# De-Rosa/PPO-BipedalWalker

Measured on AMD Instinct MI355X. Metric: env-steps/sec (whole node) + PPO-update ms, 65k walkers at 1/2/4/8 MI355X, higher is better.
Workload: dtype f32; 1 GPU; BASELINE config 4: 65536 walkers over 1 GPU(s) (65536/GPU), config 3 step: rollout T_h=64 with policy sampling + PPO update E=5, global minibatch 65536 (65536/GPU); walkers_per_gpu=65536, global_walkers=65536, horizon=64, epochs=5, minibatch_global=65536, parallelism=dp1, exchange=none

## Files before the change

### ppo-bipedalwalker_amd/csrc/wk_device.h

```cpp
#pragma once
#include <float.h>
#include "wk_common.h"
#include "wk_sincos_small.h"


namespace wk {

#define DEV __device__ __forceinline__

struct V2 { float x, y; };
typedef float pf2 __attribute__((ext_vector_type(2)));
DEV V2 mk(float x, float y) { V2 r; r.x = x; r.y = y; return r; }
DEV V2 vadd(V2 a, V2 b) { return mk(a.x + b.x, a.y + b.y); }
DEV V2 vsub(V2 a, V2 b) { return mk(a.x - b.x, a.y - b.y); }
DEV V2 vmul(V2 a, float s) { return mk(a.x * s, a.y * s); }
DEV V2 vdiv(V2 a, float d) { float f = 1.0f / d; return mk(a.x * f, a.y * f); }
DEV V2 vneg(V2 a) { return mk(-a.x, -a.y); }
DEV float vdot(V2 a, V2 b) { return a.x * b.x + a.y * b.y; }
DEV float sqrt_core(float x) {
  const float y = __builtin_amdgcn_rsqf(x);
  const float s0 = x * y;
  const float e = __builtin_fmaf(-s0, s0, x);
  return __builtin_fmaf(e, 0.5f * y, s0);
}
// ... 270 lines not shown
  constexpr int steps = L == 16 ? 4 : (L == 8 ? 3 : 2);
#pragma unroll
  for (int s = 0; s < steps; s++) {
    const int osep = dpp_i(sep, s), oidx = dpp_i(idx, s);
    const float od = dpp_f(depth, s), onx = dpp_f(nx, s), ony = dpp_f(ny, s);
    sep |= osep;
    const bool take = (od < depth) || (od == depth && oidx < idx);
    depth = take ? od : depth;
    idx = take ? oidx : idx;
    nx = take ? onx : nx;
    ny = take ? ony : ny;
  }
}

template <int NA, int NB>
DEV void edge_of(const Poly<NA>& A, const Poly<NB>& B, int k, V2& p0, V2& p1) {
  uint32_t x0 = 0u, y0 = 0u, x1 = 0u, y1 = 0u;
#pragma unroll
  for (int i = 0; i < NA + NB; i++) {
    const uint32_t m = (k == i) ? 0xffffffffu : 0u;
    const bool fa = i < NA;
    const int a = fa ? i : i - NA;
    const int b = fa ? (a + 1) % NA : (a + 1) % NB;
    const float sx = fa ? A.x[fa ? a : 0] : B.x[fa ? 0 : a];
    const float sy = fa ? A.y[fa ? a : 0] : B.y[fa ? 0 : a];
    const float ex = fa ? A.x[fa ? b : 0] : B.x[fa ? 0 : b];
    const float ey = fa ? A.y[fa ? b : 0] : B.y[fa ? 0 : b];
    x0 |= m & __float_as_uint(sx); y0 |= m & __float_as_uint(sy);
    x1 |= m & __float_as_uint(ex); y1 |= m & __float_as_uint(ey);
  }
  p0 = mk(__uint_as_float(x0), __uint_as_float(y0));
  p1 = mk(__uint_as_float(x1), __uint_as_float(y1));
}

template <int L, int NA, int NB>
DEV bool sat_row(const Poly<NA>& A, const Poly<NB>& B, int sub, V2& normal, float& depth) {
  static_assert(NA + NB <= L, "one axis per lane");
  int sep = 0, idx = 1 << 20;
  float d = FLT_MAX, nx = 0.0f, ny = 0.0f;
  if (sub < NA + NB) {
    V2 p0, p1;
    edge_of(A, B, sub, p0, p1);
    const float ex = p1.x - p0.x, ey = p1.y - p0.y;
    V2 axis = mk(-ey, ex);
    if (!(axis.x == 0.0f && axis.y == 0.0f)) {
      axis = vnormalize(axis);
      float amin, amax, bmin, bmax;
      project2(axis.x, axis.y, A, B, amin, amax, bmin, bmax);
      float temp;
      bool overlapping;
      if (sub < NA) {
        temp = net_minf(bmax - amin, amax - bmin);
        overlapping = (amin < bmax) && (bmin < amax);
      } else {
        temp = net_minf(amax - bmin, bmax - amin);
        overlapping = (bmin < amax) && (amin < bmax);
      }
      if (!overlapping) sep = 1;
      d = temp; idx = sub; nx = axis.x; ny = axis.y;
    }
  }
  row_reduce<L>(sep, d, idx, nx, ny);
  normal = idx < (1 << 20) ? mk(nx, ny) : mk(0.0f, 0.0f);
  depth = d;
  const bool result = sep == 0;
  V2 dir = mk(B.cx - A.cx, B.cy - A.cy);
  if (vdot(dir, normal) > 0.0f) normal = vmul(normal, -1.0f);
  return result;
}

template <int N>
DEV V2 pick(const Poly<N>& p, int i) {
  uint32_t bx = 0u, by = 0u;
#pragma unroll
  for (int k = 0; k < N; k++) {
    const uint32_t m = (i == k) ? 0xffffffffu : 0u;
    bx |= m & __float_as_uint(p.x[k]);
    by |= m & __float_as_uint(p.y[k]);
  }
  return mk(__uint_as_float(bx), __uint_as_float(by));
}

DEV uint32_t bsel(uint32_t m, float a, uint32_t b) { return (m & __float_as_uint(a)) | (~m & b); }
template <int N, bool SAFE = false>
DEV void significant_face(const Poly<N>& P, V2 n, V2& fa, V2& fb, V2& fmax) {
  float mind = FLT_MAX;
  uint32_t sx = 0u, sy = 0u;
  uint32_t ax = __float_as_uint(P.x[0]), ay = __float_as_uint(P.y[0]);
  uint32_t bx = __float_as_uint(P.x[N - 2]), by = __float_as_uint(P.y[N - 2]);
#pragma unroll
  for (int i = 0; i < N; i++) {
    const float p = P.x[i] * n.x + P.y[i] * n.y;
    const bool lt = p < mind;
    const uint32_t m = lt ? 0xffffffffu : 0u;
    mind = lt ? p : mind;
    sx = bsel(m, P.x[i], sx);
    sy = bsel(m, P.y[i], sy);
    ax = bsel(m, P.x[(i + 1) % N], ax);
    ay = bsel(m, P.y[(i + 1) % N], ay);
    bx = bsel(m, P.x[(i + N - 1) % N], bx);
    by = bsel(m, P.y[(i + N - 1) % N], by);
  }
  const V2 sig = mk(__uint_as_float(sx), __uint_as_float(sy));
  const V2 va = mk(__uint_as_float(ax), __uint_as_float(ay));
  const V2 vb = mk(__uint_as_float(bx), __uint_as_float(by));
  V2 after = SAFE ? vnormalize(vsub(sig, va)) : vnormalize_edge(vsub(sig, va));
  V2 before = SAFE ? vnormalize(vsub(sig, vb)) : vnormalize_edge(vsub(sig, vb));
  const bool first = vdot(n, before) >= vdot(n, after);
  fa = first ? sig : va;
  fb = first ? vb : sig;
  fmax = sig;
}

template <int N>
DEV void significant_face_ax(const Poly<N>& P, const EdgeAxes<N>& AX, V2 n, V2& fa, V2& fb,
                             V2& fmax, V2& fdir) {
  float mind = FLT_MAX;
  uint32_t sx = 0u, sy = 0u;
  uint32_t ax = __float_as_uint(P.x[0]), ay = __float_as_uint(P.y[0]);
  uint32_t bx = __float_as_uint(P.x[N - 2]), by = __float_as_uint(P.y[N - 2]);
  uint32_t ex = __float_as_uint(AX.x[N - 1]), ey = __float_as_uint(AX.y[N - 1]);
  uint32_t px = __float_as_uint(AX.x[N - 2]), py = __float_as_uint(AX.y[N - 2]);
#pragma unroll
  for (int i = 0; i < N; i++) {
    const float p = P.x[i] * n.x + P.y[i] * n.y;
    const bool lt = p < mind;
    const uint32_t m = lt ? 0xffffffffu : 0u;
    mind = lt ? p : mind;
    sx = bsel(m, P.x[i], sx);
    sy = bsel(m, P.y[i], sy);
    ax = bsel(m, P.x[(i + 1) % N], ax);
    ay = bsel(m, P.y[(i + 1) % N], ay);
    bx = bsel(m, P.x[(i + N - 1) % N], bx);
    by = bsel(m, P.y[(i + N - 1) % N], by);
    ex = bsel(m, AX.x[i], ex);
    ey = bsel(m, AX.y[i], ey);
    px = bsel(m, AX.x[(i + N - 1) % N], px);
    py = bsel(m, AX.y[(i + N - 1) % N], py);
  }
  const V2 sig = mk(__uint_as_float(sx), __uint_as_float(sy));
  const V2 va = mk(__uint_as_float(ax), __uint_as_float(ay));
  const V2 vb = mk(__uint_as_float(bx), __uint_as_float(by));
  const V2 after = mk(-__uint_as_float(ey), __uint_as_float(ex));
  const V2 before = mk(__uint_as_float(py), -__uint_as_float(px));
  const bool first = vdot(n, before) >= vdot(n, after);
  fa = first ? sig : va;
  fb = first ? vb : sig;
  fmax = sig;
  fdir = first ? vneg(before) : after;
}
template <int N, int S>
DEV void significant_face_lds(const Poly<N>& P, const EdgeAxes<N>& AX, V2 n, float4* rec, V2& fa,
                              V2& fb, V2& fmax, V2& fdir) {
#pragma unroll
  for (int k = 0; k < N; k++) rec[k * S] = make_float4(P.x[k], P.y[k], AX.x[k], AX.y[k]);
  float mind = FLT_MAX;
  int idx = -1;
#pragma unroll
  for (int i = 0; i < N; i++) {
    const float p = P.x[i] * n.x + P.y[i] * n.y;
    const bool lt = p < mind;
    mind = lt ? p : mind;
    idx = lt ? i : idx;
  }
  const int ie = idx < 0 ? N - 1 : idx;
  const int inx = idx == N - 1 ? 0 : idx + 1;
  const int ipv = idx <= 0 ? idx + N - 1 : idx - 1;
  __builtin_amdgcn_wave_barrier();
  const float4 re = rec[ie * S], rn = rec[inx * S], rp = rec[ipv * S];
  const V2 sig = idx < 0 ? mk(0.0f, 0.0f) : mk(re.x, re.y);
  const V2 va = mk(rn.x, rn.y);
  const V2 vb = mk(rp.x, rp.y);
  const V2 after = mk(-re.w, re.z);
  const V2 before = mk(rp.w, -rp.z);
  const bool first = vdot(n, before) >= vdot(n, after);
  fa = first ? sig : va;
  fb = first ? vb : sig;
  fmax = sig;
  fdir = first ? vneg(before) : after;
}

DEV EdgeAxes<4> floor_axes() {
  EdgeAxes<4> a;
  a.x[0] = 1.0f;  a.y[0] = 0.0f;
  a.x[1] = -0.0f; a.y[1] = 1.0f;
  a.x[2] = -1.0f; a.y[2] = 0.0f;
  a.x[3] = -0.0f; a.y[3] = -1.0f;
  return a;
}

DEV int clip_vectors(V2 a, V2 b, V2 n, float offset, V2& o0, V2& o1) {
  const float da = vdot(a, n) - offset;
  const float db = vdot(b, n) - offset;
  const bool ka = da >= 0.0f, kb = db >= 0.0f, kx = da * db < 0.0f;
  const float location = da / (da - db);
  const V2 edge = vadd(vmul(vsub(b, a), location), a);
  const V2 second = kb ? b : edge;
  V2 r0 = ka ? a : (kb ? b : edge);
  V2 r1 = ka ? second : edge;
  const bool has0 = ka || kb || kx;
  const bool has1 = ka ? (kb || kx) : (kb && kx);
  o0 = has0 ? r0 : o0;
  o1 = has1 ? r1 : o1;
  return (int)ka + (int)kb + (int)kx;
}

DEV int contact_clip(V2 ra, V2 rb, V2 rmax, V2 rd, V2 ia, V2 ib, V2 imax, V2 id, V2 normal,
                     V2& c0, V2& c1) {
  V2 rf = vsub(rb, ra);
  V2 iv = vsub(ib, ia);
  if (fabsf(vdot(rf, normal)) > fabsf(vdot(iv, normal))) {
    V2 t;
    t = ra; ra = ia; ia = t;
    t = rb; rb = ib; ib = t;
    t = rmax; rmax = imax; imax = t;
    rd = id;
  }
  rf = rd;
  float offset = vdot(rf, ra);
  V2 p0 = mk(0.0f, 0.0f), p1 = mk(0.0f, 0.0f);
  const int k1 = clip_vectors(ia, ib, rf, offset, p0, p1);
  offset = vdot(rf, rb);
  V2 q0 = mk(0.0f, 0.0f), q1 = mk(0.0f, 0.0f);
  const int k2 = clip_vectors(p0, p1, vneg(rf), -offset, q0, q1);
  if (k1 < 2 || k2 < 2) return 0;
  V2 refn = mk(rf.y, -rf.x);
  float maximum = vdot(refn, rmax);
  int cnt = 2;
  if (vdot(refn, q0) - maximum < 0.0f) { q0 = q1; cnt = 1; }
  V2 last = cnt == 2 ? q1 : q0;
  if (vdot(refn, last) - maximum < 0.0f) cnt = cnt == 2 ? 1 : 0;
  c0 = q0;
  c1 = q1;
  return cnt;
}
template <int NA, int NB, int S = 0>
DEV int contact_points_ax(const Poly<NA>& A, const EdgeAxes<NA>& AXA, const Poly<NB>& B,
                          const EdgeAxes<NB>& AXB, V2 normal, V2& c0, V2& c1,
                          float4* rec = nullptr) {
  V2 ra, rb, rmax, rd, ia, ib, imax, id;
  if constexpr (S > 0) {
    significant_face_lds<NA, S>(A, AXA, normal, rec, ra, rb, rmax, rd);
    __builtin_amdgcn_wave_barrier();
    significant_face_lds<NB, S>(B, AXB, vneg(normal), rec, ia, ib, imax, id);
  } else {
    significant_face_ax(A, AXA, normal, ra, rb, rmax, rd);
    significant_face_ax(B, AXB, vneg(normal), ia, ib, imax, id);
  }
  return contact_clip(ra, rb, rmax, rd, ia, ib, imax, id, normal, c0, c1);
}
DEV void floor_face_ax(V2 n, V2& fa, V2& fb, V2& fmax, V2& fdir) {
  const float xa = -50.0f * n.x, xb = 1050.0f * n.x, ya = 1050.0f * n.y, yb = 900.0f * n.y;
  const float p[4] = {xa + ya, xa + yb, xb + yb, xb + ya};
  float mind = FLT_MAX;
  bool b0 = false, b1 = false;
#pragma unroll
  for (int i = 0; i < 4; i++) {
    const bool lt = p[i] < mind;
    mind = lt ? p[i] : mind;
    b0 = lt ? (i & 1) != 0 : b0;
    b1 = lt ? (i >> 1) != 0 : b1;
  }
  const bool bx = b0 != b1;
  const V2 sig = mk(b1 ? 1050.0f : -50.0f, bx ? 900.0f : 1050.0f);
  const V2 va = mk(bx ? 1050.0f : -50.0f, b1 ? 1050.0f : 900.0f);
  const V2 vb = mk(bx ? -50.0f : 1050.0f, b1 ? 900.0f : 1050.0f);
  const float ex = b0 ? -0.0f : (b1 ? -1.0f : 1.0f), ey = b0 ? (b1 ? -1.0f : 1.0f) : 0.0f;
  const float px = b0 ? (b1 ? -1.0f : 1.0f) : -0.0f, py = b0 ? 0.0f : (b1 ? 1.0f : -1.0f);
  const V2 after = mk(-ey, ex);
  const V2 before = mk(py, -px);
  const bool first = vdot(n, before) >= vdot(n, after);
  fa = first ? sig : va;
  fb = first ? vb : sig;
  fmax = sig;
  fdir = first ? vneg(before) : after;
}
template <int NA, int S = 0>
DEV int contact_points_floor(const Poly<NA>& A, const EdgeAxes<NA>& AXA, V2 normal, V2& c0,
                             V2& c1, float4* rec = nullptr) {
  V2 ra, rb, rmax, rd, ia, ib, imax, id;
  if constexpr (S > 0) significant_face_lds<NA, S>(A, AXA, normal, rec, ra, rb, rmax, rd);
  else significant_face_ax(A, AXA, normal, ra, rb, rmax, rd);
  floor_face_ax(vneg(normal), ia, ib, imax, id);
  return contact_clip(ra, rb, rmax, rd, ia, ib, imax, id, normal, c0, c1);
}

template <int NA, int NB, bool SAFE = false>
DEV int contact_points(const Poly<NA>& A, const Poly<NB>& B, V2 normal, V2& c0, V2& c1) {
  V2 ra, rb, rmax, ia, ib, imax;
  significant_face(A, normal, ra, rb, rmax);
  V2 rf = vsub(rb, ra);
  significant_face<NB, SAFE>(B, vneg(normal), ia, ib, imax);
  V2 iv = vsub(ib, ia);
  if (fabsf(vdot(rf, normal)) > fabsf(vdot(iv, normal))) {
    V2 t;
    t = ra; ra = ia; ia = t;
    t = rb; rb = ib; ib = t;
    t = rmax; rmax = imax; imax = t;
    rf = vsub(rb, ra);
  }
  rf = SAFE ? vnormalize(rf) : vnormalize_edge(rf);
  float offset = vdot(rf, ra);
  V2 p0 = mk(0.0f, 0.0f), p1 = mk(0.0f, 0.0f);
  const int k1 = clip_vectors(ia, ib, rf, offset, p0, p1);
  offset = vdot(rf, rb);
  V2 q0 = mk(0.0f, 0.0f), q1 = mk(0.0f, 0.0f);
  const int k2 = clip_vectors(p0, p1, vneg(rf), -offset, q0, q1);
  if (k1 < 2 || k2 < 2) return 0;
  V2 refn = mk(rf.y, -rf.x);
  float maximum = vdot(refn, rmax);
  int cnt = 2;
  if (vdot(refn, q0) - maximum < 0.0f) { q0 = q1; cnt = 1; }
  V2 last = cnt == 2 ? q1 : q0;
  if (vdot(refn, last) - maximum < 0.0f) {
    cnt = cnt == 2 ? 1 : 0;
  }
  c0 = q0;
  c1 = q1;
  return cnt;
}

DEV float calc_impulse(const Body& A, const Body& B, V2 contact, float force, V2 normal, V2& rA,
                       V2& rB) {
  rA = mk(contact.x - A.cx, contact.y - A.cy);
  V2 pA = mk(-rA.y, rA.x);
  float ctcA = vdot(normal, pA);
  rB = mk(contact.x - B.cx, contact.y - B.cy);
  V2 pB = mk(-rB.y, rB.x);
  float ctcB = vdot(normal, pB);
  V2 aVel = vadd(mk(A.d->vx, A.d->vy), vmul(pA, A.d->w));
  V2 bVel = vadd(mk(B.d->vx, B.d->vy), vmul(pB, B.d->w));
  V2 vel = vsub(bVel, aVel);
  float vdn = vdot(vel, normal);
  float j = -force * vdn;
  float denom = (A.im + B.im) + ((ctcA * ctcA) * A.ii) + ((ctcB * ctcB) * B.ii);
  return j / denom;
}

template <bool BSTATIC>
DEV void apply_impulses(Body& A, Body& B, V2 normal, float impulse, V2 rA, V2 rB) {
  V2 J = vmul(normal, impulse);
  V2 va = vsub(mk(A.d->vx, A.d->vy), vmul(J, A.im));
  A.d->vx = va.x;
  A.d->vy = va.y;
  if (!BSTATIC) {
    V2 vb = vadd(mk(B.d->vx, B.d->vy), vmul(J, B.im));
    B.d->vx = vb.x;
    B.d->vy = vb.y;
  }
  V2 pA = mk(-rA.y, rA.x);
  A.d->w = A.d->w - (vdot(pA, J) * A.ii);
  if (!BSTATIC) {
    V2 pB = mk(-rB.y, rB.x);
    B.d->w = B.d->w + (vdot(pB, J) * B.ii);
  }
}

}
```

### ppo-bipedalwalker_amd/csrc/wk_physics.hip

```cpp
#include "wk_common.h"
#include "wk_device.h"
#include "wk_kernels.h"
#include "wk_mfma_layout.h"
#include "wk_region_prof.h"
#include "wk_sample.h"

#ifndef WK_PHYS_PART
#define WK_PHYS_PART 0
#endif
#define WK_PART(k) (WK_PHYS_PART == 0 || WK_PHYS_PART == (k))

#define WK_ENV_WPE __attribute__((amdgpu_waves_per_eu(2, 2)))

namespace wk {

struct EnvState {
  Poly<6> lll, llu, rll, rlu;
  Poly<5> body;
  Dyn dlll, dllu, dbody, drll, drlu;
  bool clll, cllu, cbody, crll, crlu;
  float torque[4];
  float posx, posy, prevx, prevy;
  int steps, episodes;
  bool post, terminal;
};

DEV void make_pole(Poly<6>& p, float cx, float cy) {
  float adjustment = 0.1f * 75.0f;
  float h = adjustment * 3.5f;
  p.x[0] = cx + adjustment; p.y[0] = cy + h;
  p.x[1] = cx;              p.y[1] = cy + h;
  p.x[2] = cx - adjustment; p.y[2] = cy + h;
  p.x[3] = cx - adjustment; p.y[3] = cy - h;
  p.x[4] = cx;              p.y[4] = cy - h;
  p.x[5] = cx + adjustment; p.y[5] = cy - h;
  find_centroid(p);
}

DEV void zero_dyn(Dyn& d) { d.vx = 0.0f; d.vy = 0.0f; d.w = 0.0f; d.th = 0.0f; }

DEV void make_template(EnvState& s, float dx) {
  float px = 125.0f + dx, py = 800.0f;
  s.body.x[0] = px + 20; s.body.y[0] = py + 20;
  s.body.x[1] = px;      s.body.y[1] = py + 20;
  s.body.x[2] = px - 20; s.body.y[2] = py + 20;
  s.body.x[3] = px - 20; s.body.y[3] = py - 20;
  s.body.x[4] = px + 20; s.body.y[4] = py - 20;
  find_centroid(s.body);
  make_pole(s.llu, px + 0.0f, py + 30.0f);
  make_pole(s.lll, px + 0.0f, py + 60.0f);
  make_pole(s.rlu, px + 0.0f, py + 30.0f);
  make_pole(s.rll, px + 0.0f, py + 60.0f);
  zero_dyn(s.dlll); zero_dyn(s.dllu); zero_dyn(s.dbody); zero_dyn(s.drll); zero_dyn(s.drlu);
  s.clll = s.cllu = s.cbody = s.crll = s.crlu = false;
#pragma unroll
  for (int j = 0; j < 4; j++) s.torque[j] = 0.0f;
  s.steps = 0;
  s.terminal = false;
  s.prevx = px; s.prevy = py;
  s.posx = s.body.cx; s.posy = s.body.cy;
}

template <int N>
DEV void load_poly(Poly<N>& p, const float* __restrict__ st, int b, int e, int n) {
#pragma unroll
  for (int i = 0; i < N; i++) {
    p.x[i] = st[(size_t)e * NSTATE + (b * BSTRIDE + 2 * i)];
    p.y[i] = st[(size_t)e * NSTATE + (b * BSTRIDE + 2 * i + 1)];
  }
  p.cx = st[(size_t)e * NSTATE + (b * BSTRIDE + F_CX)];
  p.cy = st[(size_t)e * NSTATE + (b * BSTRIDE + F_CY)];
}
DEV void load_dyn(Dyn& d, bool& col, const float* __restrict__ st, int b, int e, int n) {
  d.vx = st[(size_t)e * NSTATE + (b * BSTRIDE + F_VX)];
  d.vy = st[(size_t)e * NSTATE + (b * BSTRIDE + F_VY)];
  d.w = st[(size_t)e * NSTATE + (b * BSTRIDE + F_W)];
  d.th = st[(size_t)e * NSTATE + (b * BSTRIDE + F_TH)];
  col = st[(size_t)e * NSTATE + (b * BSTRIDE + F_COL)] != 0.0f;
}
template <int N>
DEV void store_body(const Poly<N>& p, const Dyn& d, bool col, float* __restrict__ st, int b, int e,
                    int n) {
// ... 23 lines not shown
  load_dyn(s.dbody, s.cbody, st, BODY, e, n);
  load_dyn(s.drll, s.crll, st, RLL, e, n);
  load_dyn(s.drlu, s.crlu, st, RLU, e, n);
#pragma unroll
  for (int j = 0; j < 4; j++) s.torque[j] = st[(size_t)e * NSTATE + (S_TORQUE + j)];
  s.posx = st[(size_t)e * NSTATE + S_POS];
  s.posy = st[(size_t)e * NSTATE + (S_POS + 1)];
  s.prevx = st[(size_t)e * NSTATE + S_PREV];
  s.prevy = st[(size_t)e * NSTATE + (S_PREV + 1)];
  s.steps = (int)st[(size_t)e * NSTATE + S_STEPS];
  s.post = st[(size_t)e * NSTATE + S_POSTRESET] != 0.0f;
  s.terminal = st[(size_t)e * NSTATE + S_TERMINAL] != 0.0f;
  s.episodes = (int)st[(size_t)e * NSTATE + S_EPISODES];
}

DEV void store_state(const EnvState& s, float* __restrict__ st, int e, int n) {
  store_body(s.lll, s.dlll, s.clll, st, LLL, e, n);
  store_body(s.llu, s.dllu, s.cllu, st, LLU, e, n);
  store_body(s.body, s.dbody, s.cbody, st, BODY, e, n);
  store_body(s.rll, s.drll, s.crll, st, RLL, e, n);
  store_body(s.rlu, s.drlu, s.crlu, st, RLU, e, n);
#pragma unroll
  for (int j = 0; j < 4; j++) st[(size_t)e * NSTATE + (S_TORQUE + j)] = s.torque[j];
  st[(size_t)e * NSTATE + S_POS] = s.posx;
  st[(size_t)e * NSTATE + (S_POS + 1)] = s.posy;
  st[(size_t)e * NSTATE + S_PREV] = s.prevx;
  st[(size_t)e * NSTATE + (S_PREV + 1)] = s.prevy;
  st[(size_t)e * NSTATE + S_STEPS] = (float)s.steps;
  st[(size_t)e * NSTATE + S_POSTRESET] = s.post ? 1.0f : 0.0f;
  st[(size_t)e * NSTATE + S_TERMINAL] = s.terminal ? 1.0f : 0.0f;
  st[(size_t)e * NSTATE + S_EPISODES] = (float)s.episodes;
}

DEV void get_obs(const EnvState& s, float o[12]) {
  o[0] = s.body.x[1] / 900.0f;
  o[1] = s.body.y[1] / 500.0f;
  o[2] = s.llu.x[2] / 900.0f;
  o[3] = s.llu.y[2] / 500.0f;
  o[4] = s.rlu.x[2] / 900.0f;
  o[5] = s.rlu.y[2] / 500.0f;
  o[6] = s.dbody.vx / 60.0f;
  o[7] = s.dbody.vy / 60.0f;
  o[8] = s.dlll.th;
  o[9] = s.dllu.th;
  o[10] = s.drll.th;
  o[11] = s.drlu.th;
}

DEV float hswap(float v) {
  return __int_as_float(__builtin_amdgcn_update_dpp(0, __float_as_int(v), 0x4E, 0xF, 0xF, false));
}
DEV float fsel(uint32_t m, float a, float b) { return __uint_as_float(bsel(m, a, __float_as_uint(b))); }
template <int N>
DEV Poly<N> psel(bool c, const Poly<N>& a, const Poly<N>& b) {
  const uint32_t m = c ? 0xffffffffu : 0u;
  Poly<N> r;
#pragma unroll
  for (int i = 0; i < N; i++) { r.x[i] = fsel(m, a.x[i], b.x[i]); r.y[i] = fsel(m, a.y[i], b.y[i]); }
  r.cx = fsel(m, a.cx, b.cx);
  r.cy = fsel(m, a.cy, b.cy);
  return r;
}
template <int N>
DEV bool sat_split(const Poly<N>& A, const Poly<N>& B, int half, V2& normal, float& depth,
                   Poly<N>& P, EdgeAxes<N>& AXP) {
  P = psel(half != 0, B, A);
  const Poly<N> Q = psel(half != 0, A, B);
  bool sep = false;
  V2 nn = mk(0.0f, 0.0f);
  float dd = FLT_MAX;
  axis_pass<N, N, false, false, N, N == 6>(P, Q, sep, nn, dd, &AXP);
  const float dd_o = hswap(dd), nx_o = hswap(nn.x), ny_o = hswap(nn.y);
  const float dA = half ? dd_o : dd, dB = half ? dd : dd_o;
  const V2 nA = half ? mk(nx_o, ny_o) : nn, nB = half ? nn : mk(nx_o, ny_o);
  const bool takeB = dB < dA;
  depth = net_minf(dA, dB);
  normal = takeB ? nB : nA;
  const V2 dir = mk(B.cx - A.cx, B.cy - A.cy);
  if (vdot(dir, normal) > 0.0f) normal = vmul(normal, -1.0f);
  return depth > 0.0f;
}
template <int N, int FS = 0>
DEV int contacts_split(const Poly<N>& P, const EdgeAxes<N>& AXP, int half, V2 normal, V2& c0,
                       V2& c1, float4* frec = nullptr) {
  V2 fa, fb, fm, fd;
  if constexpr (FS > 0) significant_face_lds<N, FS>(P, AXP, half ? vneg(normal) : normal, frec, fa, fb, fm, fd);
  else significant_face_ax(P, AXP, half ? vneg(normal) : normal, fa, fb, fm, fd);
  const V2 oa = mk(hswap(fa.x), hswap(fa.y)), ob = mk(hswap(fb.x), hswap(fb.y));
  const V2 om = mk(hswap(fm.x), hswap(fm.y)), od = mk(hswap(fd.x), hswap(fd.y));
  const bool h = half != 0;
  return contact_clip(h ? oa : fa, h ? ob : fb, h ? om : fm, h ? od : fd,
                      h ? fa : oa, h ? fb : ob, h ? fm : om, h ? fd : od, normal, c0, c1);
}
DEV bool sat_floor_split(const Poly<6>& A, const Poly<4>& F, float mnx, float mny, float mxx,
                         float mxy, int half, V2& normal, float& depth, EdgeAxes<6>& AX) {
  Poly<6> R;
  const uint32_t hm = half ? 0xffffffffu : 0u;
#pragma unroll
  for (int i = 0; i < 6; i++) {
    R.x[i] = fsel(hm, A.x[(i + 3) % 6], A.x[i]);
    R.y[i] = fsel(hm, A.y[(i + 3) % 6], A.y[i]);
  }
  R.cx = A.cx;
  R.cy = A.cy;
  bool sep = false;
  V2 nn = mk(0.0f, 0.0f);
  float dd = FLT_MAX;
  EdgeAxes<6> own;
  axis_pass<6, 4, true, false, 3, true>(R, F, sep, nn, dd, &own);
  const float dd_o = hswap(dd), nx_o = hswap(nn.x), ny_o = hswap(nn.y);
  const float d0 = half ? dd_o : dd, d1 = half ? dd : dd_o;
  const V2 n0 = half ? mk(nx_o, ny_o) : nn, n1 = half ? nn : mk(nx_o, ny_o);
  const bool take1 = d1 < d0;
  depth = net_minf(d0, d1);
  normal = take1 ? n1 : n0;
#pragma unroll
  for (int i = 0; i < 3; i++) {
    const float ox = hswap(own.x[i]), oy = hswap(own.y[i]);
    AX.x[i] = half ? ox : own.x[i];
    AX.y[i] = half ? oy : own.y[i];
    AX.x[i + 3] = half ? own.x[i] : ox;
    AX.y[i + 3] = half ? own.y[i] : oy;
  }
  floor_axis(-50.0f, 1050.0f, mnx, mxx, 1.0f, 0.0f, sep, normal, depth);
  floor_axis(900.0f, 1050.0f, mny, mxy, -0.0f, 1.0f, sep, normal, depth);
  floor_axis(-1050.0f, 50.0f, -mxx, -mnx, -1.0f, 0.0f, sep, normal, depth);
  floor_axis(-1050.0f, -900.0f, -mxy, -mny, -0.0f, -1.0f, sep, normal, depth);
  V2 dir = mk(F.cx - A.cx, F.cy - A.cy);
  if (vdot(dir, normal) > 0.0f) normal = vmul(normal, -1.0f);
  return depth > 0.0f;
}

template <int NA, int NB, bool BSTATIC, bool TRACE, int L, bool GENERIC = false, int H = 1, int FS = 0>
DEV void resolve_pair(Poly<NA>& A, Dyn& dA, const Mat& mA, Poly<NB>& B, Dyn& dB, const Mat& mB,
                      bool& colA, PairTraceDev* tr, int pi, int sub, RegionProf* rp = nullptr,
                      uint32_t* ec = nullptr, float4* frec = nullptr) {
  static_assert(H == 1 || (L == 1 && !GENERIC && NA == 6 && NB == (BSTATIC ? 4 : 6)),
                "the quad split covers leg-leg and leg-floor pairs");
  static_assert(!BSTATIC || NB == 4, "the static body is the floor");
  static_assert(!GENERIC || BSTATIC, "generic static floor polygon");
  constexpr bool FLAT = BSTATIC && !GENERIC;
  constexpr int EVK = !BSTATIC ? 0 : (NA == 5 ? 2 : 1);
  float mnx, mny, mxx, mxy;
  aabb(A, mnx, mny, mxx, mxy);
  bool ov;
  if constexpr (FLAT) {
    ov = mnx < 1050.0f && mxx > -50.0f && mny < 1050.0f && mxy > 900.0f;
  } else {
    float b0x, b0y, b1x, b1y;
    aabb(B, b0x, b0y, b1x, b1y);
    ov = mnx < b1x && mxx > b0x && mny < b1y && mxy > b0y;
  }
  rp_mark(rp, RP_AABB_LL + EVK, ov ? 1.0f : 0.0f);
  if (!ov) return;
  if (ec) ec[EV_AABB_LL + EVK]++;
  if (TRACE && tr && pi >= 0) tr->aabb_hit[pi] = 1;
  if (BSTATIC) colA = true;
  V2 n;
  float depth;
  bool hit;
  constexpr bool KEEP = L == 1 && !GENERIC;
  EdgeAxes<NA> axa;
  EdgeAxes<NB> axb;
  Poly<NA> own;
  if constexpr (H == 2 && FLAT) hit = sat_floor_split(A, B, mnx, mny, mxx, mxy, sub, n, depth, axa);
  else if constexpr (H == 2) hit = sat_split(A, B, sub, n, depth, own, axa);
  else if constexpr (L > 1) hit = sat_row<L>(A, B, sub, n, depth);
  else if constexpr (FLAT) hit = sat_floor<NA, NA == 6>(A, B, mnx, mny, mxx, mxy, n, depth, &axa);
  else if constexpr (KEEP) hit = sat<NA, NB, false, true>(A, B, n, depth, &axa, &axb);
  else hit = sat<NA, NB, GENERIC, true>(A, B, n, depth);
  rp_mark(rp, RP_SAT_LL + EVK, depth, n.x, n.y, hit ? 1.0f : 0.0f);
  if (!hit) return;
  if (ec) ec[EV_SAT_LL + EVK]++;
  V2 c0, c1;
  int nc;
  if constexpr (H == 2 && !BSTATIC) nc = contacts_split<NA, FS>(own, axa, sub, n, c0, c1, frec);
  else if constexpr (KEEP && FLAT) nc = contact_points_floor<NA, FS>(A, axa, n, c0, c1, frec);
  else if constexpr (KEEP) nc = contact_points_ax<NA, NB, FS>(A, axa, B, axb, n, c0, c1, frec);
  else nc = contact_points<NA, NB, GENERIC>(A, B, n, c0, c1);
  rp_mark(rp, RP_CON_LL + EVK, c0.x, c0.y, c1.x, c1.y, (float)nc);
  if (TRACE && tr && pi >= 0) {
    tr->sat_hit[pi] = 1;
    tr->n_contacts[pi] = (uint8_t)nc;
    tr->normal[pi][0] = n.x;
    tr->normal[pi][1] = n.y;
    tr->depth[pi] = depth;
    if (nc > 0) { tr->contact[pi][0][0] = c0.x; tr->contact[pi][0][1] = c0.y; }
    if (nc > 1) { tr->contact[pi][1][0] = c1.x; tr->contact[pi][1][1] = c1.y; }
  }
  if (BSTATIC) {
    move(A, vmul(n, depth));
  } else {
    move(A, vdiv(vmul(n, depth), 2.0f));
    move(B, vdiv(vmul(vneg(n), depth), 2.0f));
  }
  if (ec) ec[EV_CONTACTS] += (uint32_t)nc;
  if (nc == 0) return;
  if (ec) ec[EV_IMP_LL + EVK]++;
  float e = net_maxf(mA.e, mB.e);
  float mu = net_minf(mA.mu, mB.mu);
  V2 contact = nc == 2 ? vdiv(vadd(c0, c1), 2.0f) : c0;
  Body bA{A.cx, A.cy, &dA, mA.im, mA.ii};
  Body bB{B.cx, B.cy, &dB, mB.im, mB.ii};
  V2 rA, rB, rAF, rBF;
  V2 tangent = mk(-n.y, n.x);
  float j, jf;
  if constexpr (H == 2) {
    const uint32_t hm = sub ? 0xffffffffu : 0u;
    const float mine = calc_impulse(bA, bB, contact, fsel(hm, mu, 1.0f + e),
                                    mk(fsel(hm, tangent.x, n.x), fsel(hm, tangent.y, n.y)), rA, rB);
    const float other = hswap(mine);
    j = fsel(hm, other, mine);
    jf = fsel(hm, mine, other);
    rAF = rA;
    rBF = rB;
  } else {
    j = calc_impulse(bA, bB, contact, 1.0f + e, n, rA, rB);
    jf = calc_impulse(bA, bB, contact, mu, tangent, rAF, rBF);
  }
// ... 459 lines not shown
  s.posx = r[S_POS]; s.posy = r[S_POS + 1];
  s.prevx = r[S_PREV]; s.prevy = r[S_PREV + 1];
  s.steps = (int)r[S_STEPS];
  s.post = r[S_POSTRESET] != 0.0f;
  s.terminal = r[S_TERMINAL] != 0.0f;
  s.episodes = (int)r[S_EPISODES];
}

DEV void store_side(const SideState& s, float* __restrict__ st, int e, int side) {
  store_body(s.lo, s.dlo, s.clo, st, side ? RLL : LLL, e, 0);
  store_body(s.up, s.dup, s.cup, st, side ? RLU : LLU, e, 0);
  float* r = st + (size_t)e * NSTATE;
  r[S_TORQUE + side] = s.tq_up;
  r[S_TORQUE + 2 + side] = s.tq_lo;
  if (side == 0) {
    store_body(s.body, s.dbody, s.cbody, st, BODY, e, 0);
    r[S_POS] = s.posx; r[S_POS + 1] = s.posy;
    r[S_PREV] = s.prevx; r[S_PREV + 1] = s.prevy;
    r[S_STEPS] = (float)s.steps;
    r[S_POSTRESET] = s.post ? 1.0f : 0.0f;
    r[S_TERMINAL] = s.terminal ? 1.0f : 0.0f;
    r[S_EPISODES] = (float)s.episodes;
  }
}

DEV void make_template_side(SideState& s, float dx) {
  float px = 125.0f + dx, py = 800.0f;
  s.body.x[0] = px + 20; s.body.y[0] = py + 20;
  s.body.x[1] = px;      s.body.y[1] = py + 20;
  s.body.x[2] = px - 20; s.body.y[2] = py + 20;
  s.body.x[3] = px - 20; s.body.y[3] = py - 20;
  s.body.x[4] = px + 20; s.body.y[4] = py - 20;
  find_centroid(s.body);
  make_pole(s.up, px + 0.0f, py + 30.0f);
  make_pole(s.lo, px + 0.0f, py + 60.0f);
  zero_dyn(s.dlo); zero_dyn(s.dup); zero_dyn(s.dbody);
  s.clo = s.cup = s.cbody = false;
  s.tq_up = 0.0f; s.tq_lo = 0.0f;
  s.steps = 0;
  s.terminal = false;
  s.prevx = px; s.prevy = py;
  s.posx = s.body.cx; s.posy = s.body.cy;
}

DEV void get_obs_side(const SideState& s, int side, float o[12]) {
  const float ux = s.up.x[2], uy = s.up.y[2], tlo = s.dlo.th, tup = s.dup.th;
  const float oux = pswap(ux), ouy = pswap(uy), otlo = pswap(tlo), otup = pswap(tup);
  const bool left = side == 0;
  o[0] = s.body.x[1] / 900.0f;
  o[1] = s.body.y[1] / 500.0f;
  o[2] = (left ? ux : oux) / 900.0f;
  o[3] = (left ? uy : ouy) / 500.0f;
  o[4] = (left ? oux : ux) / 900.0f;
  o[5] = (left ? ouy : uy) / 500.0f;
  o[6] = s.dbody.vx / 60.0f;
  o[7] = s.dbody.vy / 60.0f;
  o[8] = left ? tlo : otlo;
  o[9] = left ? tup : otup;
  o[10] = left ? otlo : tlo;
  o[11] = left ? otup : tup;
}

template <bool TRACE, bool ROUGH, int TS>
DEV void torso_step(SideState& s, const Mat& mb, float dt, float adx, float ady, PairTraceDev* tr,
                    int side, RegionProf* rp, const float* ter) {
  integrate(s.body, s.dbody, dt, adx, ady);
  rp_mark(rp, RP_INTEG, s.body.x[0], s.body.y[3], s.dbody.th);
  if constexpr (ROUGH) {
    floor_pairs<5, TRACE, 1, true, TS>(s.body, s.dbody, mb, s.cbody, side == 0 ? tr : nullptr, 4, 0, ter);
  } else {
    Poly<4> fl;
    floor_poly(fl);
    Dyn dfl;
    zero_dyn(dfl);
    const Mat mf{0.0f, 0.0f, 0.3f, 1.0f};
    resolve_pair<5, 4, true, TRACE, 1>(s.body, s.dbody, mb, fl, dfl, mf, s.cbody,
                                       side == 0 ? tr : nullptr, 4, 0, rp);
  }
}

template <bool TRACE, int Q, bool ROUGH = false, int TS = 1, int FS = 0>
DEV void substep_side(SideState& s, const Mat& mp, const Mat& mb, float dt, float adx, float ady,
                      PairTraceDev* tr, int side, int half, RegionProf* rp, const float* ter = nullptr,
                      float4* frec = nullptr) {
  rp_mark(rp, RP_OTHER);
  Poly<4> fl;
  floor_poly(fl);
  Dyn dfl;
  zero_dyn(dfl);
  const Mat mf{0.0f, 0.0f, 0.3f, 1.0f};
  if (side == 0) joint_step<5, 6, 1, 4, TRACE>(s.body, s.dbody, mb, s.up, s.dup, mp, tr, 0);
  bcast_torso<0xA0>(s.body, s.dbody);
  if (side == 1) joint_step<5, 6, 1, 4, TRACE>(s.body, s.dbody, mb, s.up, s.dup, mp, tr, 1);
  bcast_torso<0xF5>(s.body, s.dbody);
  joint_step<6, 6, 2, 3, TRACE>(s.up, s.dup, mp, s.lo, s.dlo, mp, tr, 2 + side);
  rp_mark(rp, RP_JOINT, s.dup.w, s.dlo.w, s.up.x[0], s.lo.x[0], s.dbody.w, s.body.x[0]);
  const int pb = side ? 5 : 0;
  torso_step<TRACE, ROUGH, TS>(s, mb, dt, adx, ady, tr, side, rp, ter);
  integrate(s.lo, s.dlo, dt, adx, ady);
  rp_mark(rp, RP_INTEG, s.lo.x[0], s.lo.y[3], s.lo.x[5], s.dlo.th);
#pragma unroll
  for (int q = 0; q < 3; q++) {
    if (q == 1) resolve_pair<6, 6, false, TRACE, 1, false, Q, FS>(s.lo, s.dlo, mp, s.up, s.dup, mp, s.clo, tr, pb + 0, half, rp, nullptr, frec);
    else if ((q == 0) == s.post) {
      if constexpr (ROUGH) floor_pairs<6, TRACE, 1, true, TS>(s.lo, s.dlo, mp, s.clo, tr, pb + 1, 0, ter);
      else resolve_pair<6, 4, true, TRACE, 1, false, Q, FS>(s.lo, s.dlo, mp, fl, dfl, mf, s.clo, tr, pb + 1, half, rp, nullptr, frec);
    }
    rp_mark(rp, RP_OTHER);
  }
  integrate(s.up, s.dup, dt, adx, ady);
  rp_mark(rp, RP_INTEG, s.up.x[0], s.up.y[3], s.up.x[5], s.dup.th);
#pragma unroll
  for (int q = 0; q < 3; q++) {
    if (q == 1) resolve_pair<6, 6, false, TRACE, 1, false, Q, FS>(s.up, s.dup, mp, s.lo, s.dlo, mp, s.cup, tr, pb + 2, half, rp, nullptr, frec);
    else if ((q == 0) == s.post) {
      if constexpr (ROUGH) floor_pairs<6, TRACE, 1, true, TS>(s.up, s.dup, mp, s.cup, tr, pb + 3, 0, ter);
      else resolve_pair<6, 4, true, TRACE, 1, false, Q, FS>(s.up, s.dup, mp, fl, dfl, mf, s.cup, tr, pb + 3, half, rp, nullptr, frec);
    }
    rp_mark(rp, RP_OTHER);
  }
  rp_mark(rp, RP_OTHER);
}

DEV bool side_finite(const SideState& s) {
  const float acc = nonfinite_acc(s.lo, s.dlo) + nonfinite_acc(s.up, s.dup) + nonfinite_acc(s.body, s.dbody);
  return acc == 0.0f;
}

typedef float pf4 __attribute__((ext_vector_type(4)));
DEV uint32_t lane_opaque(uint32_t v) {
  asm volatile("" : "+v"(v));
  return v;
}
template <typename T>
DEV void st_row(T v, T* p) { *p = v; }
DEV void st_row4(float* p, float a, float b, float c, float d) {
  const pf4 v = {a, b, c, d};
  st_row(v, (pf4*)p);
}
DEV pf4 pmfma(float a, float b, pf4 c) { return __builtin_amdgcn_mfma_f32_16x16x4f32(a, b, c, 0, 0, 0); }
DEV float plrelu(float z) { return z < 0.0f ? 0.2f * z : z; }

template <int Q>
DEV void policy_mfma(const float* __restrict__ Wz, const float obs[12], bool writer,
                     float* __restrict__ pl, float z3[4], float& value, int tx) {
  using namespace mf;
  constexpr int NT = 2 / Q;
  const int lane = tx & 63, n = lane & 15, g = lane >> 4, wl = lane >> (Q == 2 ? 2 : 1);
  float* tile = pl;
  float* outs = pl + 512;
  if (writer) {
#pragma unroll
    for (int q = 0; q < 3; q++) {
      const pf4 v = {obs[4 * q], obs[4 * q + 1], obs[4 * q + 2], obs[4 * q + 3]};
      *(pf4*)(tile + wl * 16 + 4 * q) = v;
    }
  }
  wave_lds_sync();
  const pf4 z4 = {0.0f, 0.0f, 0.0f, 0.0f};
#pragma unroll 1
  for (int nt = 0; nt < NT; nt++) {
    float sB[3];
#pragma unroll
    for (int t = 0; t < 3; t++) sB[t] = tile[(16 * nt + n) * 16 + 4 * t + g];
    pf4 h1[4];
    float pv = 0.0f;
#pragma unroll
// ... 26 lines not shown
#pragma unroll
      for (int Mp = 0; Mp < 4; Mp++) {
        const pf4 w = *(const pf4*)(Wz + W2F + ((Mt * 4 + Mp) * 64 + lane) * 4);
#pragma unroll
        for (int r = 0; r < 4; r++) acc = pmfma(w[r], h1[Mp][r], acc);
      }
      const pf4 b2 = *(const pf4*)(Wz + BA2 + 16 * Mt + 4 * g);
#pragma unroll
      for (int r = 0; r < 4; r++) {
        const int k = 16 * Mt + 4 * g + r;
        const float h2 = plrelu(acc[r] + b2[r]);
#pragma unroll
        for (int d = 0; d < 4; d++) p3[d] = p3[d] + Wz[W3 + d * 64 + k] * h2;
      }
    }
    const float z3g = rows_rsum4(p3);
    pv = rows_sum4(pv);
    outs[(16 * nt + n) * 8 + g] = z3g;
    if (g == 0) outs[(16 * nt + n) * 8 + 4] = pv;
  }
  wave_lds_sync();
  const pf4 b3 = *(const pf4*)(Wz + BA3);
  const pf4 o = *(const pf4*)(outs + wl * 8);
#pragma unroll
  for (int d = 0; d < 4; d++) z3[d] = o[d] + b3[d];
  value = outs[wl * 8 + 4] + Wz[BC2];
  wave_lds_sync();
}

constexpr int SIDE_BLOCK = SIDE_BLOCK_THREADS;
template <bool POLICY, bool RECORD, bool TRACE, int Q, bool ROUGH = false>
__global__ __launch_bounds__(SIDE_BLOCK)
__attribute__((amdgpu_waves_per_eu(Q == 2 ? 1 : 2, Q == 2 ? 1 : 2)))
void k_env_side(EnvParams P, StepArgs A) {
  const int tid = blockIdx.x * blockDim.x + threadIdx.x;
  const int side = tid & 1;
  const int half = Q == 2 ? (tid >> 1) & 1 : 0;
  constexpr int SH = Q == 2 ? 2 : 1;
  const int n = P.n_env;
  const int wpw = Q == 2 ? P.wpw : 64 >> SH;
  const int eraw = ((tid >> 6) * wpw) + ((tid & ((wpw << SH) - 1)) >> SH);
  const bool active = eraw < n && (tid & 63) < (wpw << SH);
  const int slot = eraw < n ? eraw : n - 1;
  const int e = A.order ? A.order[slot] : slot;
  const bool leader = side == 0 && half == 0 && active;
  __shared__ float pol_lds[POLICY ? (SIDE_BLOCK / 64) * 768 : 1];
  __shared__ float wz_lds[POLICY ? mf::WEND : 1];
  constexpr int WPB = SIDE_BLOCK >> SH;
  __shared__ float ter_lds[ROUGH ? 11 * WPB : 1];
  constexpr int FS = (Q == 1 && !ROUGH) ? SIDE_BLOCK : 0;
  __shared__ float4 face_lds[FS ? 6 * SIDE_BLOCK : 1];
  constexpr int RS = (Q == 1 && ROUGH) ? SIDE_BLOCK : 0;
  __shared__ float4 rstash_lds[RS ? 4 * SIDE_BLOCK : 1];
  constexpr int SS = FS;
  const int wib = ((threadIdx.x >> 6) * wpw) + ((threadIdx.x & ((wpw << SH) - 1)) >> SH);
  const float* const ter = ter_lds + wib;
  if constexpr (ROUGH) {
#pragma unroll 1
    for (int i = 0; i < 11; i++)
      ter_lds[i * WPB + wib] = 800.0f + (float)terrain_draw(P.seed, (uint32_t)(P.env_offset + e), i);
  }
  if (POLICY) {
    for (int i = threadIdx.x; i < mf::WEND / 4; i += SIDE_BLOCK)
      ((pf4*)wz_lds)[i] = ((const pf4*)A.Wz)[i];
    __syncthreads();
  }
  SideState s;
  load_side(s, A.st, e, side);
  const MatConst mc = material(A.mat[e]);
  const Mat mp{mc.inv_mass, 0.001f * mc.inv_mass, mc.restitution, mc.friction};
  const Mat mb{mc.inv_mass, 0.0003f, mc.restitution, mc.friction};
  const float dt = P.dt_sub;
  const float adx = 0.0f * dt, ady = 980.0f * dt;
  uint32_t t = A.rng_t[e];
  uint32_t fault = 0;
  RP_KERNEL_BEGIN(SIDE_BLOCK / 64);

#pragma unroll 1
  for (int k = 0; k < A.k_steps; k++) {
    float a[4], lp[4], obs[12];
    if (Q == 1 && A.pace) pace_partner(A.pace, A.pace_seq, k);
    rp_mark(rp, RP_OTHER);
    const int tx = (int)lane_opaque(threadIdx.x);
    float4* const frec = face_lds + (FS ? tx : 0);
    float4* const stash = frec;
    float* const wave_pol = pol_lds + (POLICY ? (tx >> 6) * 768 : 0);
    if (POLICY) {
      get_obs_side(s, side, obs);
      if constexpr (SS != 0) {
        park_legs<SS>(s, stash);
        asm volatile("" ::: "memory");
      } else if constexpr (RS != 0) {
        park_legs<RS, 4>(s, rstash_lds + tx);
        asm volatile("" ::: "memory");
      }
      float z3[4], mean[4], v;
      policy_mfma<Q>(wz_lds, obs, side == 0 && half == 0, wave_pol, z3, v, tx);
#pragma unroll
      for (int d = 0; d < 4; d++) mean[d] = tanhf(z3[d]);
      sample_actions(P, A.lp_const, (uint32_t)P.env_offset + lane_opaque((uint32_t)e), t, mean, a, lp);
      if (RECORD && leader) {
        const size_t row = (size_t)(A.t0 + k) * n;
        const uint32_t eo = lane_opaque((uint32_t)e);
#pragma unroll
        for (int q = 0; q < 3; q++)
          st_row4(A.traj_s + row * 12 + (eo * 12u + 4u * q), obs[4 * q], obs[4 * q + 1], obs[4 * q + 2],
                  obs[4 * q + 3]);
        st_row4(A.traj_a + row * 4 + eo * 4u, a[0], a[1], a[2], a[3]);
        st_row4(A.traj_lp + row * 4 + eo * 4u, lp[0], lp[1], lp[2], lp[3]);
        st_row(v, A.traj_v + row + eo);
      }
      if constexpr (SS != 0) {
        asm volatile("" ::: "memory");
        unpark_legs<SS>(s, stash);
      } else if constexpr (RS != 0) {
        asm volatile("" ::: "memory");
        unpark_legs<RS, 4>(s, rstash_lds + tx);
      }
    } else {
#pragma unroll
      for (int d = 0; d < 4; d++) a[d] = A.actions[((size_t)k * n + e) * 4 + d];
    }
    rp_mark(rp, RP_POLICY);
    s.steps++;
    {
      const float au = clip1(side ? a[1] : a[0]), al = clip1(side ? a[3] : a[2]);
      float c = au - s.tq_up; s.tq_up = au; s.dup.w = s.dup.w + c * 5.0f;
      c = al - s.tq_lo; s.tq_lo = al; s.dlo.w = s.dlo.w + c * 5.0f;
    }
#pragma unroll 1
    for (int it = 0; it < P.iterations; it++) {
      PairTraceDev* tr = (TRACE && active && half == 0) ? A.trace + ((size_t)e * P.iterations + it) : nullptr;
      substep_side<TRACE, Q, ROUGH, WPB, FS>(s, mp, mb, dt, adx, ady, tr, side, half, rp, ter, frec);
    }
    s.prevx = s.posx; s.prevy = s.posy;
    s.posx = s.body.cx; s.posy = s.body.cy;
    const bool other_cup = pswap(s.cup ? 1.0f : 0.0f) != 0.0f;
    if (s.cbody || s.cup || other_cup) s.terminal = true;
    float reward = 0.0f;
    float dX = s.posx - s.prevx;
    float yb = s.body.y[1];
    reward = reward + ((dX > 0.0f && ((yb / 500.0f) < 1.6f)) ? dX : 0.0f);
    reward = reward - (((yb / 500.0f) > 1.65f) ? -0.1f : 0.0f);
    bool terminal = false;
    if (s.terminal || s.steps > P.max_timesteps) {
      if (s.terminal) reward -= 40.0f;
      terminal = true;
    }
    if (s.posx > 900.0f) {
      reward += 80.0f;
      terminal = true;
    }
    if (!side_finite(s)) fault |= 1u;
    const size_t krow = (size_t)k * n;
    const uint32_t eo = lane_opaque((uint32_t)e);
    if (A.pos_out && leader) {
      A.pos_out[krow * 2 + eo * 2u] = s.posx;
      A.pos_out[krow * 2 + (eo * 2u + 1u)] = s.posy;
    }
    if (terminal) {
      int ep = s.episodes + 1;
      make_template_side(s, A.dxoff[lane_opaque((uint32_t)e)]);
      s.post = true;
      s.episodes = ep;
    }
    if (A.obs_out) {
      get_obs_side(s, side, obs);
      if (leader) {
#pragma unroll
        for (int i = 0; i < 12; i++) A.obs_out[krow * 12 + (eo * 12u + i)] = obs[i];
      }
    }
    if (leader) {
      if (A.rew_out) A.rew_out[krow + eo] = reward;
      if (A.done_out) A.done_out[krow + eo] = terminal ? 1 : 0;
      if (RECORD) {
        const size_t row = (size_t)(A.t0 + k) * n;
        st_row(reward, A.traj_r + row + eo);
        st_row((uint8_t)(terminal ? 1 : 0), A.traj_d + row + eo);
      }
    }
    t++;
  }
  if (active && half == 0) store_side(s, A.st, lane_opaque((uint32_t)e), (int)(lane_opaque(threadIdx.x) & 1u));
  RP_KERNEL_END();
  fault |= (uint32_t)pswap((float)fault);
  if (leader) {
    const uint32_t eo = lane_opaque((uint32_t)e);
    A.rng_t[eo] = t;
    if (A.fault_out) A.fault_out[eo] |= fault;
  }
}

#if WK_PART(3)
__global__ void k_env_init(EnvParams P, float* st, const float* dxoff, const uint8_t* mask,
                           int post) {
  const int e = blockIdx.x * blockDim.x + threadIdx.x;
// ... 216 lines not shown
```

### ppo-bipedalwalker_amd/csrc/wk_sincos_small.h

```cpp
#ifndef WK_SINCOS_SMALL_H
#define WK_SINCOS_SMALL_H
#ifdef __HIP__
#define WK_SC_FN __host__ __device__ __forceinline__
#else
#define WK_SC_FN static inline
#include <math.h>
#endif

WK_SC_FN void wk_sincos_small(double x, double* s, double* c) {
  const double x2 = x * x;
  double ps = 1.0 / 6227020800.0;
  ps = __builtin_fma(ps, x2, -1.0 / 39916800.0);
  ps = __builtin_fma(ps, x2, 1.0 / 362880.0);
  ps = __builtin_fma(ps, x2, -1.0 / 5040.0);
  ps = __builtin_fma(ps, x2, 1.0 / 120.0);
  ps = __builtin_fma(ps, x2, -1.0 / 6.0);
  *s = __builtin_fma(x * x2, ps, x);
  double pc = -1.0 / 87178291200.0;
  pc = __builtin_fma(pc, x2, 1.0 / 479001600.0);
  pc = __builtin_fma(pc, x2, -1.0 / 3628800.0);
  pc = __builtin_fma(pc, x2, 1.0 / 40320.0);
  pc = __builtin_fma(pc, x2, -1.0 / 720.0);
  pc = __builtin_fma(pc, x2, 1.0 / 24.0);
  pc = __builtin_fma(pc, x2, -0.5);
  *c = __builtin_fma(x2, pc, 1.0);
}
#endif
```

Measured before the change: 83.81 million env-steps/s.

## Store LDS face records and leg stash as planar scalars; inline-asm sincos FMAs

Face records in LDS and the parked leg polygons move from float4-per-lane records to planar float arrays with a stride that is a multiple of 64. The intent is to let the compiler use ds_write2st64/ds_read2st64 pairs and avoid bank conflicts. contact_clip replaces its branchy swap with bitmask selects to cut divergence. The double-precision sincos polynomial now interleaves the sin and cos chains and uses inline v_fma_f64 with SGPR constants to raise ILP and avoid loading constants into VGPRs, with a plain-FMA fallback for one physics part. The inline asm adds fragility and increases the number of scalar LDS ops.

```diff
diff --git a/ppo-bipedalwalker_amd/csrc/wk_device.h b/ppo-bipedalwalker_amd/csrc/wk_device.h
--- a/ppo-bipedalwalker_amd/csrc/wk_device.h
+++ b/ppo-bipedalwalker_amd/csrc/wk_device.h
@@ -376,6 +376,9 @@
 }
 
 DEV uint32_t bsel(uint32_t m, float a, uint32_t b) { return (m & __float_as_uint(a)) | (~m & b); }
+DEV V2 vbsel(uint32_t m, V2 a, V2 b) {
+  return mk(__uint_as_float(bsel(m, a.x, __float_as_uint(b.x))), __uint_as_float(bsel(m, a.y, __float_as_uint(b.y))));
+}
 template <int N, bool SAFE = false>
 DEV void significant_face(const Poly<N>& P, V2 n, V2& fa, V2& fb, V2& fmax) {
   float mind = FLT_MAX;
@@ -444,10 +447,16 @@
   fdir = first ? vneg(before) : after;
 }
 template <int N, int S>
-DEV void significant_face_lds(const Poly<N>& P, const EdgeAxes<N>& AX, V2 n, float4* rec, V2& fa,
+DEV void significant_face_lds(const Poly<N>& P, const EdgeAxes<N>& AX, V2 n, float* rec, V2& fa,
                               V2& fb, V2& fmax, V2& fdir) {
-#pragma unroll
-  for (int k = 0; k < N; k++) rec[k * S] = make_float4(P.x[k], P.y[k], AX.x[k], AX.y[k]);
+  static_assert(S % 64 == 0, "the planes' stride in ds_write2st64_b32 units");
+#pragma unroll
+  for (int k = 0; k < N; k++) {
+    rec[(4 * k + 0) * S] = P.x[k];
+    rec[(4 * k + 1) * S] = P.y[k];
+    rec[(4 * k + 2) * S] = AX.x[k];
+    rec[(4 * k + 3) * S] = AX.y[k];
+  }
   float mind = FLT_MAX;
   int idx = -1;
 #pragma unroll
@@ -461,12 +470,17 @@
   const int inx = idx == N - 1 ? 0 : idx + 1;
   const int ipv = idx <= 0 ? idx + N - 1 : idx - 1;
   __builtin_amdgcn_wave_barrier();
-  const float4 re = rec[ie * S], rn = rec[inx * S], rp = rec[ipv * S];
-  const V2 sig = idx < 0 ? mk(0.0f, 0.0f) : mk(re.x, re.y);
-  const V2 va = mk(rn.x, rn.y);
-  const V2 vb = mk(rp.x, rp.y);
-  const V2 after = mk(-re.w, re.z);
-  const V2 before = mk(rp.w, -rp.z);
+  const float* const re = rec + ie * (4 * S);
+  const float* const rn = rec + inx * (4 * S);
+  const float* const rp = rec + ipv * (4 * S);
+  const float re_x = re[0], re_y = re[S], re_ax = re[2 * S], re_ay = re[3 * S];
+  const float rn_x = rn[0], rn_y = rn[S];
+  const float rp_x = rp[0], rp_y = rp[S], rp_ax = rp[2 * S], rp_ay = rp[3 * S];
+  const V2 sig = idx < 0 ? mk(0.0f, 0.0f) : mk(re_x, re_y);
+  const V2 va = mk(rn_x, rn_y);
+  const V2 vb = mk(rp_x, rp_y);
+  const V2 after = mk(-re_ay, re_ax);
+  const V2 before = mk(rp_ay, -rp_ax);
   const bool first = vdot(n, before) >= vdot(n, after);
   fa = first ? sig : va;
   fb = first ? vb : sig;
@@ -503,13 +517,12 @@
                      V2& c0, V2& c1) {
   V2 rf = vsub(rb, ra);
   V2 iv = vsub(ib, ia);
-  if (fabsf(vdot(rf, normal)) > fabsf(vdot(iv, normal))) {
-    V2 t;
-    t = ra; ra = ia; ia = t;
-    t = rb; rb = ib; ib = t;
-    t = rmax; rmax = imax; imax = t;
-    rd = id;
-  }
+  const uint32_t sw = fabsf(vdot(rf, normal)) > fabsf(vdot(iv, normal)) ? 0xffffffffu : 0u;
+  const V2 ra0 = ra, rb0 = rb;
+  ra = vbsel(sw, ia, ra); ia = vbsel(sw, ra0, ia);
+  rb = vbsel(sw, ib, rb); ib = vbsel(sw, rb0, ib);
+  rmax = vbsel(sw, imax, rmax);
+  rd = vbsel(sw, id, rd);
   rf = rd;
   float offset = vdot(rf, ra);
   V2 p0 = mk(0.0f, 0.0f), p1 = mk(0.0f, 0.0f);
@@ -531,7 +544,7 @@
 template <int NA, int NB, int S = 0>
 DEV int contact_points_ax(const Poly<NA>& A, const EdgeAxes<NA>& AXA, const Poly<NB>& B,
                           const EdgeAxes<NB>& AXB, V2 normal, V2& c0, V2& c1,
-                          float4* rec = nullptr) {
+                          float* rec = nullptr) {
   V2 ra, rb, rmax, rd, ia, ib, imax, id;
   if constexpr (S > 0) {
     significant_face_lds<NA, S>(A, AXA, normal, rec, ra, rb, rmax, rd);
@@ -571,12 +584,33 @@
 }
 template <int NA, int S = 0>
 DEV int contact_points_floor(const Poly<NA>& A, const EdgeAxes<NA>& AXA, V2 normal, V2& c0,
-                             V2& c1, float4* rec = nullptr) {
+                             V2& c1, float* rec = nullptr) {
   V2 ra, rb, rmax, rd, ia, ib, imax, id;
   if constexpr (S > 0) significant_face_lds<NA, S>(A, AXA, normal, rec, ra, rb, rmax, rd);
   else significant_face_ax(A, AXA, normal, ra, rb, rmax, rd);
   floor_face_ax(vneg(normal), ia, ib, imax, id);
   return contact_clip(ra, rb, rmax, rd, ia, ib, imax, id, normal, c0, c1);
+}
+
+template <int S>
+DEV void park_legs_planes(const Poly<6>& lo, const Poly<6>& up, float* r) {
+#pragma unroll
+  for (int i = 0; i < 6; i++) {
+    r[i * S] = lo.x[i];
+    r[(6 + i) * S] = lo.y[i];
+    r[(12 + i) * S] = up.x[i];
+    r[(18 + i) * S] = up.y[i];
+  }
+}
+template <int S>
+DEV void unpark_legs_planes(Poly<6>& lo, Poly<6>& up, const float* r) {
+#pragma unroll
+  for (int i = 0; i < 6; i++) {
+    lo.x[i] = r[i * S];
+    lo.y[i] = r[(6 + i) * S];
+    up.x[i] = r[(12 + i) * S];
+    up.y[i] = r[(18 + i) * S];
+  }
 }
 
 template <int NA, int NB, bool SAFE = false>
diff --git a/ppo-bipedalwalker_amd/csrc/wk_physics.hip b/ppo-bipedalwalker_amd/csrc/wk_physics.hip
--- a/ppo-bipedalwalker_amd/csrc/wk_physics.hip
+++ b/ppo-bipedalwalker_amd/csrc/wk_physics.hip
@@ -1,3 +1,7 @@
+
+#if defined(WK_PHYS_PART) && WK_PHYS_PART == 5
+#define WK_SC_PLAIN_FMA 1
+#endif
 #include "wk_common.h"
 #include "wk_device.h"
 #include "wk_kernels.h"
@@ -187,7 +191,7 @@
 }
 template <int N, int FS = 0>
 DEV int contacts_split(const Poly<N>& P, const EdgeAxes<N>& AXP, int half, V2 normal, V2& c0,
-                       V2& c1, float4* frec = nullptr) {
+                       V2& c1, float* frec = nullptr) {
   V2 fa, fb, fm, fd;
   if constexpr (FS > 0) significant_face_lds<N, FS>(P, AXP, half ? vneg(normal) : normal, frec, fa, fb, fm, fd);
   else significant_face_ax(P, AXP, half ? vneg(normal) : normal, fa, fb, fm, fd);
@@ -239,7 +243,7 @@
 template <int NA, int NB, bool BSTATIC, bool TRACE, int L, bool GENERIC = false, int H = 1, int FS = 0>
 DEV void resolve_pair(Poly<NA>& A, Dyn& dA, const Mat& mA, Poly<NB>& B, Dyn& dB, const Mat& mB,
                       bool& colA, PairTraceDev* tr, int pi, int sub, RegionProf* rp = nullptr,
-                      uint32_t* ec = nullptr, float4* frec = nullptr) {
+                      uint32_t* ec = nullptr, float* frec = nullptr) {
   static_assert(H == 1 || (L == 1 && !GENERIC && NA == 6 && NB == (BSTATIC ? 4 : 6)),
                 "the quad split covers leg-leg and leg-floor pairs");
   static_assert(!BSTATIC || NB == 4, "the static body is the floor");
@@ -865,7 +869,7 @@
 template <bool TRACE, int Q, bool ROUGH = false, int TS = 1, int FS = 0>
 DEV void substep_side(SideState& s, const Mat& mp, const Mat& mb, float dt, float adx, float ady,
                       PairTraceDev* tr, int side, int half, RegionProf* rp, const float* ter = nullptr,
-                      float4* frec = nullptr) {
+                      float* frec = nullptr) {
   rp_mark(rp, RP_OTHER);
   Poly<4> fl;
   floor_poly(fl);
@@ -1058,13 +1062,13 @@
     if (Q == 1 && A.pace) pace_partner(A.pace, A.pace_seq, k);
     rp_mark(rp, RP_OTHER);
     const int tx = (int)lane_opaque(threadIdx.x);
-    float4* const frec = face_lds + (FS ? tx : 0);
-    float4* const stash = frec;
+    float* const frec = (float*)face_lds + (FS ? tx : 0);
+    float* const stash = frec;
     float* const wave_pol = pol_lds + (POLICY ? (tx >> 6) * 768 : 0);
     if (POLICY) {
       get_obs_side(s, side, obs);
       if constexpr (SS != 0) {
-        park_legs<SS>(s, stash);
+        park_legs_planes<SS>(s.lo, s.up, stash);
         asm volatile("" ::: "memory");
       } else if constexpr (RS != 0) {
         park_legs<RS, 4>(s, rstash_lds + tx);
@@ -1088,7 +1092,7 @@
       }
       if constexpr (SS != 0) {
         asm volatile("" ::: "memory");
-        unpark_legs<SS>(s, stash);
+        unpark_legs_planes<SS>(s.lo, s.up, stash);
       } else if constexpr (RS != 0) {
         asm volatile("" ::: "memory");
         unpark_legs<RS, 4>(s, rstash_lds + tx);
diff --git a/ppo-bipedalwalker_amd/csrc/wk_sincos_small.h b/ppo-bipedalwalker_amd/csrc/wk_sincos_small.h
--- a/ppo-bipedalwalker_amd/csrc/wk_sincos_small.h
+++ b/ppo-bipedalwalker_amd/csrc/wk_sincos_small.h
@@ -7,6 +7,36 @@
 #include <math.h>
 #endif
 
+#if defined(__HIP_DEVICE_COMPILE__) && defined(__AMDGCN__) && !defined(WK_SC_PLAIN_FMA)
+WK_SC_FN double wk_sc_step(double p, double x2, double k) {
+  double r;
+  __asm__("v_fma_f64 %0, %1, %2, %3" : "=v"(r) : "v"(p), "v"(x2), "s"(k));
+  return r;
+}
+WK_SC_FN double wk_sc_first(double k0, double x2, double k1) {
+  double r;
+  __asm__("v_fma_f64 %0, %1, %2, %3" : "=v"(r) : "s"(k0), "v"(x2), "v"(k1));
+  return r;
+}
+WK_SC_FN void wk_sincos_small(double x, double* s, double* c) {
+  const double x2 = x * x;
+  double pc = -1.0 / 87178291200.0;
+  double ps = 1.0 / 6227020800.0;
+  pc = wk_sc_first(pc, x2, 1.0 / 479001600.0);
+  ps = wk_sc_first(ps, x2, -1.0 / 39916800.0);
+  pc = wk_sc_step(pc, x2, -1.0 / 3628800.0);
+  ps = wk_sc_step(ps, x2, 1.0 / 362880.0);
+  pc = wk_sc_step(pc, x2, 1.0 / 40320.0);
+  ps = wk_sc_step(ps, x2, -1.0 / 5040.0);
+  pc = wk_sc_step(pc, x2, -1.0 / 720.0);
+  ps = wk_sc_step(ps, x2, 1.0 / 120.0);
+  pc = wk_sc_step(pc, x2, 1.0 / 24.0);
+  ps = wk_sc_step(ps, x2, -1.0 / 6.0);
+  pc = __builtin_fma(pc, x2, -0.5);
+  *s = __builtin_fma(x * x2, ps, x);
+  *c = __builtin_fma(x2, pc, 1.0);
+}
+#else
 WK_SC_FN void wk_sincos_small(double x, double* s, double* c) {
   const double x2 = x * x;
   double ps = 1.0 / 6227020800.0;
@@ -26,3 +56,4 @@
   *c = __builtin_fma(x2, pc, 1.0);
 }
 #endif
+#endif
```

After: 85.49 million env-steps/s, median of 6. +2.0%, better.
